# songlab-cal/CherryML

Hardware: AMD Instinct MI355X
Metric: cherry-pairs/sec (whole node) per EM iter (higher is better)
Workload: dtype f64

## Files before the change

### cherryml_amd/csrc/tbasis.hip.h

```cpp
#pragma once
#include "cb_internal.hip.h"
#include "common.hip.h"
#include <hip/hip_ext.h>

namespace tbasis {

typedef long double ld;

static inline ld g_phi2(ld x) {
  if (fabsl(x) < 0.5L) {
    ld p = 1.0L;
    for (int k = 24; k >= 3; --k) p = 1.0L + p * x / (ld)k;
    return 0.5L * p;
  }
  return (expm1l(x) - x) / (x * x);
}

static inline ld dot4(const ld *a, const ld *b, int n) {
  ld s0 = 0.0L, s1 = 0.0L, s2 = 0.0L, s3 = 0.0L;
  int i = 0;
  for (; i + 3 < n; i += 4) {
    s0 += a[i] * b[i];
    s1 += a[i + 1] * b[i + 1];
    s2 += a[i + 2] * b[i + 2];
    s3 += a[i + 3] * b[i + 3];
  }
  for (; i < n; ++i) s0 += a[i] * b[i];
  return (s0 + s1) + (s2 + s3);
}

static int id_rows(int B, int N, const std::vector<ld> &F, int Rmax, ld tol, std::vector<int> &skel, std::vector<ld> &L, ld &resid) {
  std::vector<ld> W(F), Q((size_t)Rmax * N, 0.0L), Cq((size_t)B * Rmax, 0.0L), q(N);
  skel.clear();
  ld scale = 0.0L;
  int R = 0;
  bool done = false;
  for (int r = 0; r <= Rmax; ++r) {
    int p = -1;
    ld best = -1.0L;
    for (int b = 0; b < B; ++b) {
      const ld *w = &W[(size_t)b * N];
      const ld s = dot4(w, w, N);
      if (s > best) best = s, p = b;
    }
    if (r == 0) scale = sqrtl(best);
    if (!(scale > 0.0L) || sqrtl(best) <= tol * scale) {
      done = true;
      break;
    }
    if (r == Rmax) break;
    const ld inv = 1.0L / sqrtl(best);
    for (int i = 0; i < N; ++i) q[i] = W[(size_t)p * N + i] * inv;
    for (int pass = 0; pass < 2; ++pass) {
      for (int k = 0; k < r; ++k) {
        const ld *qk = &Q[(size_t)k * N];
        const ld d = dot4(qk, q.data(), N);
        for (int i = 0; i < N; ++i) q[i] -= d * qk[i];
      }
      const ld s = dot4(q.data(), q.data(), N);
      const ld in = 1.0L / sqrtl(s);
      for (int i = 0; i < N; ++i) q[i] *= in;
    }
    for (int i = 0; i < N; ++i) Q[(size_t)r * N + i] = q[i];
    for (int b = 0; b < B; ++b) {
      ld *w = &W[(size_t)b * N];
      const ld c = dot4(w, q.data(), N);
      Cq[(size_t)b * Rmax + r] = c;
      for (int i = 0; i < N; ++i) w[i] -= c * q[i];
    }
    skel.push_back(p);
    R = r + 1;
  }
  if (!done) return -1;
  L.assign((size_t)B * std::max(R, 1), 0.0L);
  for (int r = R - 1; r >= 0; --r) {
    const ld trr = Cq[(size_t)skel[r] * Rmax + r];
    for (int b = 0; b < B; ++b) {
      ld s = Cq[(size_t)b * Rmax + r];
      for (int k = r + 1; k < R; ++k) s -= L[(size_t)b * R + k] * Cq[(size_t)skel[k] * Rmax + r];
      L[(size_t)b * R + r] = s / trr;
    }
  }
  for (int r = 0; r < R; ++r)
    for (int k = 0; k < R; ++k) L[(size_t)skel[r] * R + k] = k == r ? 1.0L : 0.0L;
  resid = 0.0L;
  for (int b = 0; b < B; ++b)
    for (int i = 0; i < N; ++i) {
      ld s = F[(size_t)b * N + i];
      for (int k = 0; k < R; ++k) s -= L[(size_t)b * R + k] * F[(size_t)skel[k] * N + i];
      resid = std::max(resid, fabsl(s));
    }
  return R;
}

}

#ifndef CB_TB_SAMPLES
#define CB_TB_SAMPLES 512
#endif
#ifndef CB_TB_TOL_G
#define CB_TB_TOL_G 2e-15L
#endif
#ifndef CB_TB_X_SMALL
#define CB_TB_X_SMALL 8.0
#endif

bool cb_tb_build(int B, const double *t, double rho_max, CbTimeBasisHost &out) {
  using namespace tbasis;
  out = CbTimeBasisHost{};
  if (B < 1 || !(rho_max > 0.0) || !std::isfinite(rho_max)) return false;
  for (int b = 0; b < B; ++b)
    if (!(t[b] > 0.0) || !std::isfinite(t[b])) return false;
  const int N = CB_TB_SAMPLES + 1;
  std::vector<ld> mu(N);
  mu[0] = 0.0L;
  for (int i = 1; i < N; ++i) mu[i] = -(ld)rho_max * powl(10.0L, -6.0L + 6.0L * (ld)(i - 1) / (ld)(N - 2));
  out.B = B;
  out.rho_max = rho_max;
  for (int b = 1; b < B; ++b)
    if (!(t[b] >= t[b - 1])) return false;
  out.kind.assign(B, -1);
  std::vector<int> small_idx;
  for (int b = 0; b < B; ++b) {
    if (t[b] * rho_max <= CB_TB_X_SMALL) small_idx.push_back(b);
    else {
      out.kind[b] = (int)out.direct.size();
      out.direct.push_back(b);
    }
  }
  out.Ls.assign((size_t)B * CB_TB_RS_MAX, 0.0);
  out.Lg.assign((size_t)B * CB_TB_RG_MAX, 0.0);
  const int nsm = (int)small_idx.size();
  if (nsm > 0) {
    std::vector<ld> F((size_t)nsm * N);
    for (int k = 0; k < nsm; ++k)
      for (int i = 0; i < N; ++i) F[(size_t)k * N + i] = mu[i] * mu[i] * g_phi2((ld)t[small_idx[k]] * mu[i]);
    std::vector<int> sk;
    std::vector<ld> L;
    ld res = 0.0L;
    const int R = id_rows(nsm, N, F, std::min(CB_TB_RS_MAX, nsm), 1e-17L, sk, L, res);
    if (R < 0) return false;
    out.ns = R;
    out.res_s = (double)res;
    for (int r = 0; r < R; ++r) out.skel_s.push_back(small_idx[sk[r]]);
    for (int k = 0; k < nsm; ++k)
      for (int r = 0; r < R; ++r) out.Ls[(size_t)small_idx[k] * CB_TB_RS_MAX + r] = (double)L[(size_t)k * R + r];
  }
  out.nd = (int)out.direct.size();
  {
    std::vector<ld> F((size_t)B * N);
    for (int b = 0; b < B; ++b)
      for (int i = 0; i < N; ++i) F[(size_t)b * N + i] = expl((ld)t[b] * mu[i]);
    std::vector<int> sk;
    std::vector<ld> L;
    ld res = 0.0L;
    const int R = id_rows(B, N, F, std::min(CB_TB_RG_MAX, B), CB_TB_TOL_G, sk, L, res);
    if (R < 0) return false;
    out.ng = R;
    out.res_g = (double)res;
    out.skel_g = sk;
    for (int b = 0; b < B; ++b)
      for (int r = 0; r < R; ++r)
        out.Lg[(size_t)b * CB_TB_RG_MAX + r] = (double)(L[(size_t)b * R + r] * (ld)t[b] / (ld)t[sk[r]]);
  }
  for (int r = 0; r < out.ns; ++r) out.tf.push_back(t[out.skel_s[r]]);
  for (int r = 0; r < out.nd; ++r) out.tf.push_back(t[out.direct[r]]);
  for (int r = 0; r < out.ng; ++r) out.tg.push_back(t[out.skel_g[r]]);
  return true;
}

__global__ void tb_tables(int LD, int ns, int nd, int ng, const double *__restrict__ tf, const double *__restrict__ tg,
                          const double *__restrict__ lam, double *__restrict__ F, double *__restrict__ E, double *__restrict__ H,
                          const unsigned long long *skip) {
  if (skip && *skip != 0ull) return;
  const int idx = blockIdx.x * blockDim.x + threadIdx.x;
  const int nf = ns + nd;
  if (idx >= (nf + ng) * LD) return;
  const int r = idx / LD, k = idx - r * LD;
  if (r < nf) {
    const double t = tf[r], x = t * lam[k];
    F[idx] = r < ns ? phi2(x) / (t * t) : exp(x);
  } else {
    const double x = tg[r - nf] * lam[k];
    E[idx - nf * LD] = exp(x);
    H[idx - nf * LD] = exp(0.5 * x);
  }
}

template <int RS, int RG>
struct TbEwLds {
  static constexpr int SS = RS + 1, SG = RG + 2;
  int BP, LS, LG, TT, LT, RED, TOTAL;
  __host__ __device__ explicit TbEwLds(int B) {
    BP = (B + 15) & ~15;
    LS = 0;
    LG = LS + BP * SS;
    TT = LG + BP * SG;
    LT = TT + BP;
    RED = LT + 256;
    TOTAL = RED + 16;
  }
};

template <int RS, int RG>
__device__ __forceinline__ void tb_ew_step(int b0, int j, int k, int nsm, const double *sLs, const double *sLg, const double *sT,
                                           const double *ltab, const double (&psi)[RS / 4], double a_e, double dl, double inv_n,
                                           const double (&c)[4], const double (&pd)[4], d4 (&D)[RG / 16], double &loss, int &bad) {
  typedef TbEwLds<RS, RG> Lds;
  const bool any_small = b0 < nsm, any_direct = b0 + 16 > nsm;
  double P[4];
  if (any_small) {
    d4 acc = {0.0, 0.0, 0.0, 0.0};
#ifndef TB_NO_FWD
#pragma unroll
    for (int q = 0; q < RS / 4; ++q) acc = mfma_f64(sLs[(b0 + j) * Lds::SS + 4 * q + k], psi[q], acc);
#endif
#pragma unroll
    for (int m = 0; m < 4; ++m) {
      const double t = sT[b0 + k + 4 * m];
      P[m] = fma(t, fma(t, acc[m], a_e), dl);
    }
    if (any_direct) {
#pragma unroll
      for (int m = 0; m < 4; ++m) P[m] = (b0 + k + 4 * m < nsm) ? P[m] : pd[m];
    }
  } else {
#pragma unroll
    for (int m = 0; m < 4; ++m) P[m] = pd[m];
  }
  double g[4];
#pragma unroll
  for (int m = 0; m < 4; ++m) {
    const double cv = c[m];
    bad |= (!(P[m] >= 1e-300) && cv != 0.0) ? 1 : 0;
    const double Pu = fmax(P[m], 1e-300);
#ifdef TB_NO_LOG
    loss = fma(-cv, Pu, loss);
    g[m] = (-cv * inv_n) * Pu;
#else
    loss = fma(-cv, fast_log_table_unchecked(Pu, ltab), loss);
    g[m] = (-cv * inv_n) * fast_rcp(Pu);
#endif
  }
#ifdef TB_NO_BWD
#pragma unroll
  for (int m = 0; m < 4; ++m) D[0][m] += g[m];
#else
#pragma unroll
  for (int m = 0; m < 4; ++m) {
    const double *w = sLg + (b0 + 4 * m + k) * Lds::SG + j;
#pragma unroll
    for (int q = 0; q < RG / 16; ++q) D[q] = mfma_f64(w[16 * q], g[m], D[q]);
  }
#endif
}

template <int RS, int RG, int NWAVE, bool SYM>
__global__ __launch_bounds__(NWAVE * 64, 4) void tb_ew(CbTbEwArgs a) {
  constexpr int NT = NWAVE * 64;
  typedef TbEwLds<RS, RG> Lds;
  extern __shared__ double smem[];
  if (a.skip && *a.skip != 0ull) return;
  const Lds o(a.B);
  double *sLs = smem + o.LS, *sLg = smem + o.LG, *sT = smem + o.TT, *ltab = smem + o.LT, *sred = smem + o.RED;
  const int tid = threadIdx.x;
  for (int i = tid; i < o.BP * RS; i += NT) {
    const int b = i / RS, r = i - b * RS;
    sLs[b * Lds::SS + r] = b < a.B ? a.Ls[(size_t)b * CB_TB_RS_MAX + r] : 0.0;
  }
  for (int i = tid; i < o.BP * RG; i += NT) {
    const int b = i / RG, r = i - b * RG;
    sLg[b * Lds::SG + r] = (b < a.B && r < CB_TB_RG_MAX) ? a.Lg[(size_t)b * CB_TB_RG_MAX + r] : 0.0;
  }
  for (int i = tid; i < o.BP; i += NT) sT[i] = i < a.B ? a.t[i] : 0.0;
  fast_log_table_fill(ltab, tid, NT);
  __syncthreads();
  const size_t LL = (size_t)a.LD * a.LD;
  const int wave = tid >> 6, lane = tid & 63, j = lane & 15, k = lane >> 4;
  size_t e;
  bool live;
  double lossw = 1.0;
  if (SYM) {
    const int nb = a.LD / 16, item = (int)blockIdx.x * NWAVE + wave, blk = item >> 4, rr = item & 15;
    int I = 0, rest = blk;
    while (I < nb && rest >= nb - I) {
      rest -= nb - I;
      ++I;
    }
    live = I < nb;
    const int J = I + rest;
    e = live ? ((size_t)(16 * I + rr) * a.LD + 16 * J + j) : 0;
    lossw = J > I ? 2.0 : 1.0;
  } else {
    e = ((size_t)blockIdx.x * NWAVE + wave) * 16 + j;
    live = e < LL;
  }
  const size_t ec = live ? e : 0;
  const int row = (int)(ec / a.LD), col = (int)(ec - (size_t)row * a.LD);
  const double *__restrict__ Psi = a.Psi + ec;
  double psi[RS / 4];
#pragma unroll
  for (int q = 0; q < RS / 4; ++q) psi[q] = (4 * q + k < a.ns) ? Psi[(size_t)(4 * q + k) * LL] : 0.0;
  const double a_e = a.A[ec], dl = row == col ? 1.0 : 0.0;
  d4 D[RG / 16];
#pragma unroll
  for (int q = 0; q < RG / 16; ++q) D[q] = d4{0.0, 0.0, 0.0, 0.0};
  double loss = 0.0;
  int bad = 0;
  const int nsm = a.nsmall, B = a.B;
  const unsigned plane = (unsigned)(LL * sizeof(double));
  const __amdgpu_buffer_rsrc_t rc = __builtin_amdgcn_make_buffer_rsrc(const_cast<double *>(a.Ct), 0, 0x7fffffff, 0x00027000);
  const __amdgpu_buffer_rsrc_t rp = __builtin_amdgcn_make_buffer_rsrc(const_cast<double *>(a.Psi + (size_t)a.ns * LL), 0, 0x7fffffff, 0x00027000);
  const int eoff = (int)(ec * sizeof(double));
  int voff[4];
#pragma unroll
  for (int m = 0; m < 4; ++m) voff[m] = (int)((unsigned)(k + 4 * m) * plane) + eoff;
  auto load = [&](int b0, double (&cc)[4], double (&pp)[4]) {
    if (b0 >= B) return;
#ifdef TB_NO_LOAD
    for (int m = 0; m < 4; ++m) cc[m] = 1.0 + b0 + m, pp[m] = 0.5;
    return;
#endif
    if (b0 + 16 <= B) {
#pragma unroll
      for (int m = 0; m < 4; ++m)
        cc[m] = __builtin_bit_cast(double, __builtin_amdgcn_raw_buffer_load_b64(rc, voff[m], (int)((unsigned)b0 * plane), 0));
      if (b0 >= nsm) {
#pragma unroll
        for (int m = 0; m < 4; ++m)
          pp[m] = __builtin_bit_cast(double, __builtin_amdgcn_raw_buffer_load_b64(rp, voff[m], (int)((unsigned)(b0 - nsm) * plane), 0));
        return;
      }
      if (b0 + 16 <= nsm) return;
    } else {
#pragma unroll
      for (int m = 0; m < 4; ++m) {
        const bool in = b0 + k + 4 * m < B;
        const double v = __builtin_bit_cast(double, __builtin_amdgcn_raw_buffer_load_b64(rc, in ? voff[m] + (int)((unsigned)b0 * plane) : eoff, 0, 0));
        cc[m] = in ? v : 0.0;
      }
    }
#pragma unroll
    for (int m = 0; m < 4; ++m) {
      const int b = b0 + k + 4 * m;
      const bool in = b >= nsm && b < B;
      const double v = __builtin_bit_cast(double, __builtin_amdgcn_raw_buffer_load_b64(rp, (int)((unsigned)(in ? b - nsm : 0) * plane) + eoff, 0, 0));
      pp[m] = in ? v : 1.0;
    }
  };
  double c0[4] = {0.0, 0.0, 0.0, 0.0}, c1[4] = {0.0, 0.0, 0.0, 0.0}, p0[4] = {1.0, 1.0, 1.0, 1.0}, p1[4] = {1.0, 1.0, 1.0, 1.0};
  load(0, c0, p0);
  for (int b0 = 0; b0 < B; b0 += 32) {
    load(b0 + 16, c1, p1);
    tb_ew_step<RS, RG>(b0, j, k, nsm, sLs, sLg, sT, ltab, psi, a_e, dl, a.inv_n, c0, p0, D, loss, bad);
    if (b0 + 16 >= B) break;
    load(b0 + 32, c0, p0);
    tb_ew_step<RS, RG>(b0 + 16, j, k, nsm, sLs, sLg, sT, ltab, psi, a_e, dl, a.inv_n, c1, p1, D, loss, bad);
  }
  if (live) {
    if (a.Gh32) {
      float *__restrict__ Gh = a.Gh32 + e;
#pragma unroll
      for (int q = 0; q < RG / 16; ++q)
#pragma unroll
        for (int r = 0; r < 4; ++r) {
          const int rr = 16 * q + k + 4 * r;
          if (rr < a.ng) Gh[(size_t)rr * LL] = (float)D[q][r];
        }
    } else {
      double *__restrict__ Gh = a.Gh + e;
#pragma unroll
      for (int q = 0; q < RG / 16; ++q)
#pragma unroll
        for (int r = 0; r < 4; ++r) {
          const int rr = 16 * q + k + 4 * r;
          if (rr < a.ng) Gh[(size_t)rr * LL] = D[q][r];
        }
    }
  } else {
    loss = 0.0;
    bad = 0;
  }
  if (bad) loss = NAN;
  loss = wave_sum(loss) * lossw;
  if (lane == 0) sred[wave] = loss;
  __syncthreads();
  if (tid == 0) {
    double s = 0.0;
    for (int w = 0; w < NWAVE; ++w) s += sred[w];
    a.loss_part[blockIdx.x] = s;
  }
}

template <typename T>
__global__ __launch_bounds__(256) void tb_mirror(int LD, T *__restrict__ Gh, const unsigned long long *skip) {
  __shared__ T tile[16][17];
  if (skip && *skip != 0ull) return;
  const int nb = LD / 16;
  int I = 0, rest = (int)blockIdx.x;
  while (rest >= nb - 1 - I) {
    rest -= nb - 1 - I;
    ++I;
  }
  const int J = I + 1 + rest, r = threadIdx.x >> 4, c = threadIdx.x & 15;
  T *G = Gh + (size_t)blockIdx.y * LD * LD;
  tile[r][c] = G[(size_t)(16 * I + r) * LD + 16 * J + c];
  __syncthreads();
  G[(size_t)(16 * J + r) * LD + 16 * I + c] = tile[c][r];
}

int cb_tb_launch_tables(int LD, int ns, int nd, int ng, const double *tf, const double *tg, const double *lam, double *F, double *E,
                        double *H, const unsigned long long *skip, hipStream_t stream) {
  const int n = (ns + nd + ng) * LD;
  hipLaunchKernelGGL(tb_tables, dim3((unsigned)((n + 255) / 256)), dim3(256), 0, stream, LD, ns, nd, ng, tf, tg, lam, F, E, H, skip);
  return hipGetLastError() == hipSuccess ? 0 : -1;
}

bool cb_tb_supported(int B, int LD, int ns, int ng) {
  return ns <= CB_TB_RS_MAX && ng <= CB_TB_RG_MAX && LD % 16 == 0 && cb_tb_ew_lds_bytes(B, ns, ng) <= CB_TB_LDS_MAX &&
         (double)(B + 32) * (double)LD * (double)LD * 8.0 < 2147483648.0;
}

size_t cb_tb_ew_lds_bytes(int B, int ns, int ng) {
  const int RS = ns <= 16 ? 16 : 24, RG = ng <= 32 ? 32 : 48;
  const int BP = (B + 15) & ~15;
  return ((size_t)BP * (RS + 1 + RG + 2 + 1) + 256 + 16) * sizeof(double);
}

int cb_tb_prepare_ew(int B, int ns, int ng, size_t *cache) {
#define TB_PREP(RS_, RG_, slot_)                                                                                         \
  do {                                                                                                                   \
    const size_t lds = (size_t)TbEwLds<RS_, RG_>(B).TOTAL * sizeof(double);                                              \
    if (lds > cache[slot_]) {                                                                                            \
      if (hipFuncSetAttribute(reinterpret_cast<const void *>(tb_ew<RS_, RG_, 8, true>), hipFuncAttributeMaxDynamicSharedMemorySize, (int)lds) != hipSuccess) { \
        (void)hipGetLastError();                                                                                         \
        return -1;                                                                                                       \
      }                                                                                                                  \
      cache[slot_] = lds;                                                                                                \
    }                                                                                                                    \
  } while (0)
  if (ns <= 16 && ng <= 32) TB_PREP(16, 32, 0);
  else if (ns <= 16) TB_PREP(16, 48, 1);
  else if (ng <= 32) TB_PREP(24, 32, 2);
  else TB_PREP(24, 48, 3);
#undef TB_PREP
  return 0;
}

int cb_tb_launch_ew(const CbTbEwArgs &a, hipStream_t stream, hipEvent_t stop, int *nparts) {
  if (!cb_tb_supported(a.B, a.LD, a.ns, a.ng)) return -1;
  const int nb = a.LD / 16, nblk = nb * (nb + 1) / 2;
  const unsigned grid = (unsigned)(nblk * 2);
  if (nparts) *nparts = (int)grid;
#define TB_GO(RS_, RG_)                                                                                                  \
  do {                                                                                                                   \
    const size_t lds = (size_t)TbEwLds<RS_, RG_>(a.B).TOTAL * sizeof(double);                                            \
    hipLaunchKernelGGL((tb_ew<RS_, RG_, 8, true>), dim3(grid), dim3(512), lds, stream, a);                               \
  } while (0)
  if (a.ns <= 16 && a.ng <= 32) TB_GO(16, 32);
  else if (a.ns <= 16) TB_GO(16, 48);
  else if (a.ng <= 32) TB_GO(24, 32);
  else TB_GO(24, 48);
#undef TB_GO
  if (nb > 1) {
    const dim3 mg((unsigned)(nb * (nb - 1) / 2), (unsigned)a.ng);
    if (a.Gh32) {
      if (stop) hipExtLaunchKernelGGL(tb_mirror<float>, mg, dim3(256), 0, stream, nullptr, stop, 0, a.LD, a.Gh32, a.skip);
      else hipLaunchKernelGGL(tb_mirror<float>, mg, dim3(256), 0, stream, a.LD, a.Gh32, a.skip);
    } else {
      if (stop) hipExtLaunchKernelGGL(tb_mirror<double>, mg, dim3(256), 0, stream, nullptr, stop, 0, a.LD, a.Gh, a.skip);
      else hipLaunchKernelGGL(tb_mirror<double>, mg, dim3(256), 0, stream, a.LD, a.Gh, a.skip);
    }
  } else if (stop) {
    (void)hipEventRecord(stop, stream);
  }
  return hipGetLastError() == hipSuccess ? 0 : -1;
}
```

Baseline: 1.561 billion.

## Specialize tb_ew loop into short/direct/tail phases and batch mirror planes

The batch loop in tb_ew is split into phases: pure-short steps that load only counts, a boundary step, pure-direct steps that load counts and direct probabilities, and a partial tail. Each phase uses a templated step specialization, which removes per-step branching and lets sched_barrier keep the prefetch of the next step ahead of the compute. The LDS fill is moved after the psi and A loads and unrolled by 8 so the global loads overlap. tb_mirror now handles 8 gradient planes per block to cut launch and index overhead. In exchange the code is more complex, and the tail masking logic has changed.

New measurement: 1.578 billion, median of 6. +1.1%, better.

```diff
diff --git a/cherryml_amd/csrc/tbasis.hip.h b/cherryml_amd/csrc/tbasis.hip.h
--- a/cherryml_amd/csrc/tbasis.hip.h
+++ b/cherryml_amd/csrc/tbasis.hip.h
@@ -202,12 +202,16 @@
   }
 };
 
-template <int RS, int RG>
-__device__ __forceinline__ void tb_ew_step(int b0, int j, int k, int nsm, const double *sLs, const double *sLg, const double *sT,
-                                           const double *ltab, const double (&psi)[RS / 4], double a_e, double dl, double inv_n,
-                                           const double (&c)[4], const double (&pd)[4], d4 (&D)[RG / 16], double &loss, int &bad) {
+enum { TB_SHORT = 0, TB_DIRECT = 1, TB_ANY = 2 };
+
+template <int RS, int RG, int KIND>
+__device__ __forceinline__ void tb_ew_step(int b0, int nl, int B, int j, int k, int nsm, const double *sLs, const double *sLg,
+                                           const double *sT, const double *ltab, const double (&psi)[RS / 4], double a_e, double dl,
+                                           double inv_n, const double (&c)[4], const double (&pd)[4], d4 (&D)[RG / 16], double &loss,
+                                           int &bad) {
   typedef TbEwLds<RS, RG> Lds;
-  const bool any_small = b0 < nsm, any_direct = b0 + 16 > nsm;
+  const bool any_small = KIND == TB_SHORT || (KIND == TB_ANY && b0 < nsm);
+  const bool any_direct = KIND == TB_DIRECT || (KIND == TB_ANY && b0 + 16 > nsm);
   double P[4];
   if (any_small) {
     d4 acc = {0.0, 0.0, 0.0, 0.0};
@@ -222,16 +226,20 @@
     }
     if (any_direct) {
 #pragma unroll
-      for (int m = 0; m < 4; ++m) P[m] = (b0 + k + 4 * m < nsm) ? P[m] : pd[m];
+      for (int m = 0; m < 4; ++m) {
+        const int b = b0 + k + 4 * m;
+        P[m] = b < nsm ? P[m] : (b < B ? pd[m] : 1.0);
+      }
     }
   } else {
 #pragma unroll
-    for (int m = 0; m < 4; ++m) P[m] = pd[m];
-  }
-  double g[4];
+    for (int m = 0; m < 4; ++m) P[m] = (KIND == TB_ANY && b0 + k + 4 * m >= B) ? 1.0 : pd[m];
+  }
+  double g[4] = {0.0, 0.0, 0.0, 0.0};
 #pragma unroll
   for (int m = 0; m < 4; ++m) {
-    const double cv = c[m];
+    if (KIND == TB_ANY && m >= nl) continue;
+    const double cv = (KIND == TB_ANY && b0 + k + 4 * m >= B) ? 0.0 : c[m];
     bad |= (!(P[m] >= 1e-300) && cv != 0.0) ? 1 : 0;
     const double Pu = fmax(P[m], 1e-300);
 #ifdef TB_NO_LOG
@@ -248,11 +256,30 @@
 #else
 #pragma unroll
   for (int m = 0; m < 4; ++m) {
+    if (KIND == TB_ANY && m >= nl) continue;
     const double *w = sLg + (b0 + 4 * m + k) * Lds::SG + j;
 #pragma unroll
     for (int q = 0; q < RG / 16; ++q) D[q] = mfma_f64(w[16 * q], g[m], D[q]);
   }
 #endif
+}
+
+template <int R, int RMAX, int STRIDE, int NT>
+__device__ __forceinline__ void tb_fill_rows(double *dst, const double *__restrict__ src, int B, int BP, int tid) {
+  constexpr int U = 8;
+  for (int i0 = tid; i0 < BP * R; i0 += U * NT) {
+    double v[U];
+#pragma unroll
+    for (int u = 0; u < U; ++u) {
+      const int i = i0 + u * NT, b = i / R, r = i - b * R;
+      v[u] = (b < B && r < RMAX) ? src[(size_t)b * RMAX + r] : 0.0;
+    }
+#pragma unroll
+    for (int u = 0; u < U; ++u) {
+      const int i = i0 + u * NT, b = i / R, r = i - b * R;
+      if (i < BP * R) dst[b * STRIDE + r] = v[u];
+    }
+  }
 }
 
 template <int RS, int RG, int NWAVE, bool SYM>
@@ -264,17 +291,6 @@
   const Lds o(a.B);
   double *sLs = smem + o.LS, *sLg = smem + o.LG, *sT = smem + o.TT, *ltab = smem + o.LT, *sred = smem + o.RED;
   const int tid = threadIdx.x;
-  for (int i = tid; i < o.BP * RS; i += NT) {
-    const int b = i / RS, r = i - b * RS;
-    sLs[b * Lds::SS + r] = b < a.B ? a.Ls[(size_t)b * CB_TB_RS_MAX + r] : 0.0;
-  }
-  for (int i = tid; i < o.BP * RG; i += NT) {
-    const int b = i / RG, r = i - b * RG;
-    sLg[b * Lds::SG + r] = (b < a.B && r < CB_TB_RG_MAX) ? a.Lg[(size_t)b * CB_TB_RG_MAX + r] : 0.0;
-  }
-  for (int i = tid; i < o.BP; i += NT) sT[i] = i < a.B ? a.t[i] : 0.0;
-  fast_log_table_fill(ltab, tid, NT);
-  __syncthreads();
   const size_t LL = (size_t)a.LD * a.LD;
   const int wave = tid >> 6, lane = tid & 63, j = lane & 15, k = lane >> 4;
   size_t e;
@@ -302,6 +318,11 @@
 #pragma unroll
   for (int q = 0; q < RS / 4; ++q) psi[q] = (4 * q + k < a.ns) ? Psi[(size_t)(4 * q + k) * LL] : 0.0;
   const double a_e = a.A[ec], dl = row == col ? 1.0 : 0.0;
+  tb_fill_rows<RS, CB_TB_RS_MAX, Lds::SS, NT>(sLs, a.Ls, a.B, o.BP, tid);
+  tb_fill_rows<RG, CB_TB_RG_MAX, Lds::SG, NT>(sLg, a.Lg, a.B, o.BP, tid);
+  for (int i = tid; i < o.BP; i += NT) sT[i] = i < a.B ? a.t[i] : 0.0;
+  fast_log_table_fill(ltab, tid, NT);
+  __syncthreads();
   d4 D[RG / 16];
 #pragma unroll
   for (int q = 0; q < RG / 16; ++q) D[q] = d4{0.0, 0.0, 0.0, 0.0};
@@ -315,48 +336,101 @@
   int voff[4];
 #pragma unroll
   for (int m = 0; m < 4; ++m) voff[m] = (int)((unsigned)(k + 4 * m) * plane) + eoff;
-  auto load = [&](int b0, double (&cc)[4], double (&pp)[4]) {
-    if (b0 >= B) return;
+  auto load_c = [&](int b0, double (&cc)[4]) {
 #ifdef TB_NO_LOAD
-    for (int m = 0; m < 4; ++m) cc[m] = 1.0 + b0 + m, pp[m] = 0.5;
+    for (int m = 0; m < 4; ++m) cc[m] = 1.0 + b0 + m;
     return;
 #endif
-    if (b0 + 16 <= B) {
-#pragma unroll
-      for (int m = 0; m < 4; ++m)
-        cc[m] = __builtin_bit_cast(double, __builtin_amdgcn_raw_buffer_load_b64(rc, voff[m], (int)((unsigned)b0 * plane), 0));
-      if (b0 >= nsm) {
-#pragma unroll
-        for (int m = 0; m < 4; ++m)
-          pp[m] = __builtin_bit_cast(double, __builtin_amdgcn_raw_buffer_load_b64(rp, voff[m], (int)((unsigned)(b0 - nsm) * plane), 0));
-        return;
-      }
-      if (b0 + 16 <= nsm) return;
-    } else {
-#pragma unroll
-      for (int m = 0; m < 4; ++m) {
-        const bool in = b0 + k + 4 * m < B;
-        const double v = __builtin_bit_cast(double, __builtin_amdgcn_raw_buffer_load_b64(rc, in ? voff[m] + (int)((unsigned)b0 * plane) : eoff, 0, 0));
-        cc[m] = in ? v : 0.0;
-      }
+#pragma unroll
+    for (int m = 0; m < 4; ++m)
+      cc[m] = __builtin_bit_cast(double, __builtin_amdgcn_raw_buffer_load_b64(rc, voff[m], (int)((unsigned)b0 * plane), 0));
+  };
+  auto load_p = [&](int b0, double (&pp)[4]) {
+#ifdef TB_NO_LOAD
+    for (int m = 0; m < 4; ++m) pp[m] = 0.5;
+    return;
+#endif
+#pragma unroll
+    for (int m = 0; m < 4; ++m)
+      pp[m] = __builtin_bit_cast(double, __builtin_amdgcn_raw_buffer_load_b64(rp, voff[m], (int)((unsigned)(b0 - nsm) * plane), 0));
+  };
+  auto load_any = [&](int b0, double (&cc)[4], double (&pp)[4]) {
+#ifdef TB_NO_LOAD
+    for (int m = 0; m < 4; ++m) cc[m] = b0 + k + 4 * m < B ? 1.0 + b0 + m : 0.0, pp[m] = 0.5;
+    return;
+#endif
+#pragma unroll
+    for (int m = 0; m < 4; ++m) {
+      const bool in = b0 + k + 4 * m < B;
+      const double v = __builtin_bit_cast(double, __builtin_amdgcn_raw_buffer_load_b64(rc, in ? voff[m] + (int)((unsigned)b0 * plane) : eoff, 0, 0));
+      cc[m] = v;
     }
 #pragma unroll
     for (int m = 0; m < 4; ++m) {
       const int b = b0 + k + 4 * m;
       const bool in = b >= nsm && b < B;
       const double v = __builtin_bit_cast(double, __builtin_amdgcn_raw_buffer_load_b64(rp, (int)((unsigned)(in ? b - nsm : 0) * plane) + eoff, 0, 0));
-      pp[m] = in ? v : 1.0;
+      pp[m] = v;
     }
   };
-  double c0[4] = {0.0, 0.0, 0.0, 0.0}, c1[4] = {0.0, 0.0, 0.0, 0.0}, p0[4] = {1.0, 1.0, 1.0, 1.0}, p1[4] = {1.0, 1.0, 1.0, 1.0};
-  load(0, c0, p0);
-  for (int b0 = 0; b0 < B; b0 += 32) {
-    load(b0 + 16, c1, p1);
-    tb_ew_step<RS, RG>(b0, j, k, nsm, sLs, sLg, sT, ltab, psi, a_e, dl, a.inv_n, c0, p0, D, loss, bad);
-    if (b0 + 16 >= B) break;
-    load(b0 + 32, c0, p0);
-    tb_ew_step<RS, RG>(b0 + 16, j, k, nsm, sLs, sLg, sT, ltab, psi, a_e, dl, a.inv_n, c1, p1, D, loss, bad);
-  }
+  const int nA = (nsm < B ? nsm : B) >> 4, sC = (nsm + 15) >> 4, nF = B >> 4;
+  auto load_step = [&](int s, double (&cc)[4], double (&pp)[4]) {
+    if (s >= sC && s < nF) {
+      load_c(16 * s, cc);
+      load_p(16 * s, pp);
+    } else if (16 * s < B) {
+      load_any(16 * s, cc, pp);
+    }
+  };
+#define TB_STEP(KIND_, s_, nl_) \
+  tb_ew_step<RS, RG, KIND_>(16 * (s_), nl_, B, j, k, nsm, sLs, sLg, sT, ltab, psi, a_e, dl, a.inv_n, cc, pp, D, loss, bad)
+#define TB_NEXT()                 \
+  do {                            \
+    _Pragma("unroll") for (int m = 0; m < 4; ++m) cc[m] = cn[m], pp[m] = pn[m]; \
+  } while (0)
+  double cc[4] = {0.0, 0.0, 0.0, 0.0}, cn[4] = {0.0, 0.0, 0.0, 0.0}, pp[4] = {1.0, 1.0, 1.0, 1.0}, pn[4] = {1.0, 1.0, 1.0, 1.0};
+  int s = 0;
+  if (nA > 0) {
+    load_c(0, cc);
+    for (; s + 1 < nA; ++s) {
+      load_c(16 * (s + 1), cn);
+      __builtin_amdgcn_sched_barrier(0);
+      TB_STEP(TB_SHORT, s, 4);
+#pragma unroll
+      for (int m = 0; m < 4; ++m) cc[m] = cn[m];
+    }
+    load_step(nA, cn, pn);
+    __builtin_amdgcn_sched_barrier(0);
+    TB_STEP(TB_SHORT, s, 4);
+    TB_NEXT();
+    ++s;
+  } else {
+    load_step(0, cc, pp);
+  }
+  if (s < sC && s < nF) {
+    load_step(s + 1, cn, pn);
+    __builtin_amdgcn_sched_barrier(0);
+    TB_STEP(TB_ANY, s, 4);
+    TB_NEXT();
+    ++s;
+  }
+  if (s < nF) {
+    for (; s + 1 < nF; ++s) {
+      load_c(16 * (s + 1), cn);
+      load_p(16 * (s + 1), pn);
+      __builtin_amdgcn_sched_barrier(0);
+      TB_STEP(TB_DIRECT, s, 4);
+      TB_NEXT();
+    }
+    load_step(nF, cn, pn);
+    __builtin_amdgcn_sched_barrier(0);
+    TB_STEP(TB_DIRECT, s, 4);
+    TB_NEXT();
+    ++s;
+  }
+  if (16 * s < B) TB_STEP(TB_ANY, s, (B - 16 * s + 3) >> 2);
+#undef TB_STEP
+#undef TB_NEXT
   if (live) {
     if (a.Gh32) {
       float *__restrict__ Gh = a.Gh32 + e;
@@ -392,9 +466,10 @@
   }
 }
 
+#define TB_MIRROR_R 8
 template <typename T>
-__global__ __launch_bounds__(256) void tb_mirror(int LD, T *__restrict__ Gh, const unsigned long long *skip) {
-  __shared__ T tile[16][17];
+__global__ __launch_bounds__(256) void tb_mirror(int LD, int ng, T *__restrict__ Gh, const unsigned long long *skip) {
+  __shared__ T tile[TB_MIRROR_R][16][17];
   if (skip && *skip != 0ull) return;
   const int nb = LD / 16;
   int I = 0, rest = (int)blockIdx.x;
@@ -403,10 +478,19 @@
     ++I;
   }
   const int J = I + 1 + rest, r = threadIdx.x >> 4, c = threadIdx.x & 15;
-  T *G = Gh + (size_t)blockIdx.y * LD * LD;
-  tile[r][c] = G[(size_t)(16 * I + r) * LD + 16 * J + c];
+  const size_t LL = (size_t)LD * LD;
+  const int r0 = (int)blockIdx.y * TB_MIRROR_R, nr = ng - r0 < TB_MIRROR_R ? ng - r0 : TB_MIRROR_R;
+  T *G = Gh + (size_t)r0 * LL;
+  const size_t src = (size_t)(16 * I + r) * LD + 16 * J + c, dst = (size_t)(16 * J + r) * LD + 16 * I + c;
+  T v[TB_MIRROR_R];
+#pragma unroll
+  for (int q = 0; q < TB_MIRROR_R; ++q) v[q] = q < nr ? G[(size_t)q * LL + src] : T(0);
+#pragma unroll
+  for (int q = 0; q < TB_MIRROR_R; ++q) tile[q][r][c] = v[q];
   __syncthreads();
-  G[(size_t)(16 * J + r) * LD + 16 * I + c] = tile[c][r];
+#pragma unroll
+  for (int q = 0; q < TB_MIRROR_R; ++q)
+    if (q < nr) G[(size_t)q * LL + dst] = tile[q][c][r];
 }
 
 int cb_tb_launch_tables(int LD, int ns, int nd, int ng, const double *tf, const double *tg, const double *lam, double *F, double *E,
@@ -463,13 +547,13 @@
   else TB_GO(24, 48);
 #undef TB_GO
   if (nb > 1) {
-    const dim3 mg((unsigned)(nb * (nb - 1) / 2), (unsigned)a.ng);
+    const dim3 mg((unsigned)(nb * (nb - 1) / 2), (unsigned)((a.ng + TB_MIRROR_R - 1) / TB_MIRROR_R));
     if (a.Gh32) {
-      if (stop) hipExtLaunchKernelGGL(tb_mirror<float>, mg, dim3(256), 0, stream, nullptr, stop, 0, a.LD, a.Gh32, a.skip);
-      else hipLaunchKernelGGL(tb_mirror<float>, mg, dim3(256), 0, stream, a.LD, a.Gh32, a.skip);
+      if (stop) hipExtLaunchKernelGGL(tb_mirror<float>, mg, dim3(256), 0, stream, nullptr, stop, 0, a.LD, a.ng, a.Gh32, a.skip);
+      else hipLaunchKernelGGL(tb_mirror<float>, mg, dim3(256), 0, stream, a.LD, a.ng, a.Gh32, a.skip);
     } else {
-      if (stop) hipExtLaunchKernelGGL(tb_mirror<double>, mg, dim3(256), 0, stream, nullptr, stop, 0, a.LD, a.Gh, a.skip);
-      else hipLaunchKernelGGL(tb_mirror<double>, mg, dim3(256), 0, stream, a.LD, a.Gh, a.skip);
+      if (stop) hipExtLaunchKernelGGL(tb_mirror<double>, mg, dim3(256), 0, stream, nullptr, stop, 0, a.LD, a.ng, a.Gh, a.skip);
+      else hipLaunchKernelGGL(tb_mirror<double>, mg, dim3(256), 0, stream, a.LD, a.ng, a.Gh, a.skip);
     }
   } else if (stop) {
     (void)hipEventRecord(stop, stream);
```
